# hku-mars/loam_livox

Measured on AMD Instinct MI355X. Metric: scans_per_s, higher is better.
Workload: dtype f32 points / f64 solve; 1 GPU; C2: 24k-pt Mid-40 scan vs 5M-pt corner+surface map, 10 ICP iters (fixed), k=5, Q-full; scan_points=24000, map_points=4975193, map_corner=995155, map_surf=3980038, icp_iters=10, distinct_scans_in_batch=256

## Files before the change

### loam_livox_amd/csrc/ll_reg_kernels.hip

```cpp
#include <hip/hip_runtime.h>
#include <stdlib.h>

#include "ll_reg_query.h"
#include "ll_reg_solve_common.h"

namespace ll {

#define RQ_THREADS 256
#define RQ_WAVES (RQ_THREADS / 64)
#ifndef RS_PREFETCH
#define RS_PREFETCH 2
#endif
#define RS_WAVES (RS_THREADS / 64)
#define HASH_EMPTY 0xffffffffffffffffull


#ifndef LL_REG_MAPS_TU

__global__ __launch_bounds__(KB_THREADS) void reg_transform_kernel(RegDev rd, RegConst rc, int skip_kinds)
{
    const int b = blockIdx.y, kind = blockIdx.z;
    if ((skip_kinds >> kind) & 1) return;
    const RegState *st = rd.state + b;
    if (st->done) return;
// ... 429 lines not shown
#define FAST_MAXK (FAST_MAX_BLOCKS / RS_THREADS)
#define HT_SIZE 16384
#define HT_PART 6144
#define DD_BM_WORDS 16384
#define DD_CB_LOG2 11
#define DD_CB_SIZE (1 << DD_CB_LOG2)
#define DD_EX_SIZE 4096
#define DD_MAX_COLL 900
#define DD2_WORDS 16384
#define DD2_SLOTS (DD2_WORDS * 16)
#define DD2B_WORDS 8192
#define DD2B_SLOTS (DD2B_WORDS * 16)
#define DD2_LIST 2048
#define SEL_BINS 4096
#define SEL_CAND 1024


template <int NK>
__device__ __forceinline__ void inlier_threshold_regs(const double (&l1r)[NK], int total, unsigned long long *s_table, SolveShared &sh,
                                                      const RegConst &rc)
{
    static_assert(NK <= 64 && NK <= FAST_MAXK, "register tile of the fast paths (one bit per entry in the 64-bit masks)");
    const int tid = threadIdx.x;
    LL_T0(t_dd);
    unsigned long long first_mask = 0;
    {
        int my = 0;
        unsigned int *bmA = (unsigned int *)s_table;
        unsigned int *bmB = bmA + DD2_WORDS;
        unsigned long long *dl = (unsigned long long *)(bmB + DD2B_WORDS);
        {
            uint4 *z = (uint4 *)s_table;
            for (int e = tid; e < (DD2_WORDS + DD2B_WORDS) / 4; e += RS_THREADS) z[e] = make_uint4(0u, 0u, 0u, 0u);
            if (tid == 0) sh.n_cand = 0;
        }
        __syncthreads();
        const int kt = (total + RS_THREADS - 1) / RS_THREADS;
        auto slot_a = [](unsigned long long key) -> unsigned int {
            unsigned int h = (unsigned int)key * 0x9E3779B1u;
            h ^= h >> 15;
            h += (unsigned int)(key >> 32) * 0x85EBCA77u;
            h ^= h >> 13;
            return h & (DD2_SLOTS - 1);
        };
        auto slot_b = [](unsigned long long key) -> unsigned int {
            unsigned int h2 = ((unsigned int)(key >> 32) * 0xC2B2AE3Du) ^ ((unsigned int)key * 0x27D4EB2Fu);
            return (h2 ^ (h2 >> 16)) & (DD2B_SLOTS - 1);
        };
        unsigned long long valid_mask = 0, cont_mask = 0;
#pragma unroll
        for (int k = 0; k < NK; k++) {
            if (k >= kt) continue;
            const double l1 = l1r[k];
            const bool valid = l1 >= 0.0;
            const unsigned int slot = slot_a((unsigned long long)__double_as_longlong(l1));
            const unsigned int bit0 = valid ? (1u << ((slot & 15u) * 2u)) : 0u;
            const unsigned int old = atomicOr(&bmA[slot >> 4], bit0);
            atomicOr(&bmA[slot >> 4], (old & bit0) << 1);
            if (valid) valid_mask |= 1ull << k;
        }
        __syncthreads();
#pragma unroll
        for (int k = 0; k < NK; k++) {
            if (k >= kt) continue;
            const unsigned long long key = (unsigned long long)__double_as_longlong(l1r[k]);
            const unsigned int slot = slot_a(key);
            const bool contested = ((valid_mask >> k) & 1ull) && ((bmA[slot >> 4] >> ((slot & 15u) * 2u)) & 2u);
            const unsigned int h2 = slot_b(key);
            const unsigned int bit0 = contested ? (1u << ((h2 & 15u) * 2u)) : 0u;
            const unsigned int old = atomicOr(&bmB[h2 >> 4], bit0);
            atomicOr(&bmB[h2 >> 4], (old & bit0) << 1);
            if (contested) cont_mask |= 1ull << k;
        }
        __syncthreads();
        unsigned long long twice_mask = 0;
#pragma unroll
        for (int k = 0; k < NK; k++) {
            if (k >= kt) continue;
            const unsigned int h2 = slot_b((unsigned long long)__double_as_longlong(l1r[k]));
            if (((cont_mask >> k) & 1ull) && ((bmB[h2 >> 4] >> ((h2 & 15u) * 2u)) & 2u)) twice_mask |= 1ull << k;
        }
        my = __popcll(valid_mask & ~twice_mask);
        first_mask = valid_mask & ~twice_mask;
        int my_pos[2] = {-1, -1};
        int n_twice = __popcll(twice_mask);
        if (twice_mask) {
            int got = 0;
#pragma unroll
            for (int k = 0; k < NK; k++) {
                if (!((twice_mask >> k) & 1ull)) continue;
                const int pos = atomicAdd(&sh.n_cand, 1);
                if (pos < DD2_LIST) dl[pos] = (unsigned long long)__double_as_longlong(l1r[k]);
                if (got < 2) my_pos[got] = pos;
                got++;
            }
        }
        const int over = block_sum_int(n_twice > 2 ? 1 : 0, sh);
        const int n_list = sh.n_cand;
        if (n_list <= DD2_LIST && over == 0) {
            if (twice_mask) {
                int got = 0;
#pragma unroll
                for (int k = 0; k < NK; k++) {
                    if (!((twice_mask >> k) & 1ull)) continue;
                    const int pos = my_pos[got < 2 ? got : 1];
                    got++;
                    const unsigned long long key = (unsigned long long)__double_as_longlong(l1r[k]);
                    bool dup = false;
                    for (int j = 0; j < pos; j++) dup |= (dl[j] == key);
                    if (!dup) {
                        first_mask |= 1ull << k;
                        my++;
                    }
                }
            }
        } else {
            first_mask = 0;
            my = 0;
            const int rounds = (total + HT_PART - 1) / HT_PART;
            for (int rnd = 0; rnd < rounds; rnd++) {
                __syncthreads();
                for (int e = tid; e < HT_SIZE; e += RS_THREADS) s_table[e] = HASH_EMPTY;
                __syncthreads();
#pragma unroll
                for (int k = 0; k < NK; k++) {
                    const double l1 = l1r[k];
                    if (!(l1 >= 0.0)) continue;
                    const unsigned long long key = (unsigned long long)__double_as_longlong(l1);
                    const unsigned long long hk = hash64(key);
                    if ((int)((hk >> 40) % (unsigned long long)rounds) != rnd) continue;
                    unsigned int h = (unsigned int)hk & (HT_SIZE - 1);
                    for (;;) {
                        const unsigned long long old = atomicCAS(&s_table[h], HASH_EMPTY, key);
                        if (old == HASH_EMPTY) {
                            first_mask |= (1ull << k);
                            my++;
                            break;
                        }
                        if (old == key) break;
                        h = (h + 1u) & (HT_SIZE - 1);
                    }
                }
            }
        }
        const int nu = block_sum_int(my, sh);
        if (tid == 0) {
            sh.n_unique = nu;
            sh.sel_prefix = 0ull;
            int target = (int)(rc.inlier_ratio * (double)nu);
            if (target > nu - 1) target = nu - 1;
            sh.sel_rank = target;
        }
        __syncthreads();
    }
    LL_TACC(3, t_dd);
    LL_T0(t_sel);
    if (sh.n_unique > 0) {
        int *bins = (int *)s_table;
        unsigned long long *cand = s_table + SEL_BINS / 2;
        double kmin = INFINITY, kmax = -INFINITY;
#pragma unroll
        for (int k = 0; k < NK; k++)
            if (first_mask & (1ull << k)) {
                kmin = fmin(kmin, l1r[k]);
                kmax = fmax(kmax, l1r[k]);
            }
        for (int off = 32; off > 0; off >>= 1) {
            kmin = fmin(kmin, __shfl_down(kmin, off));
            kmax = fmax(kmax, __shfl_down(kmax, off));
        }
        if ((tid & 63) == 0) {
            sh.red[tid >> 6][0] = kmin;
            sh.red[tid >> 6][1] = kmax;
        }
        for (int e = tid; e < SEL_BINS; e += RS_THREADS) bins[e] = 0;
        __syncthreads();
        double lo = sh.red[0][0], hi = sh.red[0][1];
        for (int w = 1; w < RS_WAVES; w++) {
            lo = fmin(lo, sh.red[w][0]);
            hi = fmax(hi, sh.red[w][1]);
        }
        const double scale = (hi > lo) ? (double)(SEL_BINS - 1) / (hi - lo) : 0.0;
#pragma unroll
        for (int k = 0; k < NK; k++)
            if (first_mask & (1ull << k)) {
                int bi = (int)((l1r[k] - lo) * scale);
                bi = bi < 0 ? 0 : (bi > SEL_BINS - 1 ? SEL_BINS - 1 : bi);
                atomicAdd(&bins[bi], 1);
            }
        __syncthreads();
        {
            const int per = SEL_BINS / RS_THREADS;
            const int lane = tid & 63, wave = tid >> 6;
            int part = 0;
            for (int e = 0; e < per; e++) part += bins[tid * per + e];
            int incl = part;
#pragma unroll
            for (int off = 1; off < 64; off <<= 1) {
                const int y = __shfl_up(incl, off);
                if (lane >= off) incl += y;
            }
            if (lane == 63) sh.isum[wave] = incl;
            if (tid == 0) sh.n_cand = 0;
            __syncthreads();
            int below = incl - part;
            for (int w = 0; w < wave; w++) below += sh.isum[w];
            const int rank = sh.sel_rank;
            __syncthreads();
            const bool last_thread = tid == RS_THREADS - 1;
            if ((rank >= below && rank < below + part) || (last_thread && rank >= below + part)) {
                int cum = below, bi = tid * per;
                for (; bi < tid * per + per - 1; bi++) {
                    if (cum + bins[bi] > rank) break;
                    cum += bins[bi];
                }
                sh.sel_bin = bi;
                sh.sel_rank = rank - cum;
                sh.sel_cnt = bins[bi];
            }
            __syncthreads();
        }
        if (sh.sel_cnt <= SEL_CAND) {
            const int sel_bin = sh.sel_bin;
#pragma unroll
            for (int k = 0; k < NK; k++)
                if (first_mask & (1ull << k)) {
                    int bi = (int)((l1r[k] - lo) * scale);
                    bi = bi < 0 ? 0 : (bi > SEL_BINS - 1 ? SEL_BINS - 1 : bi);
                    if (bi == sel_bin) cand[atomicAdd(&sh.n_cand, 1)] = (unsigned long long)__double_as_longlong(l1r[k]);
                }
            __syncthreads();
            const int m = sh.n_cand;
            for (int i = tid; i < m; i += RS_THREADS) {
                const unsigned long long ki = cand[i];
                int rk = 0;
                for (int j = 0; j < m; j++) rk += (cand[j] < ki) ? 1 : 0;
                if (rk == sh.sel_rank) sh.sel_prefix = ki;
            }
            __syncthreads();
        } else {
            const int sel_bin = sh.sel_bin;
            if (tid == 0) sh.sel_prefix = 0ull;
            __syncthreads();
            for (int pass = 0; pass < 8; pass++) {
                const int shift = 56 - 8 * pass;
                for (int e = tid; e < 256; e += RS_THREADS) sh.hist[e] = 0;
                __syncthreads();
                const unsigned long long prefix = sh.sel_prefix;
#pragma unroll
                for (int k = 0; k < NK; k++) {
                    if (!(first_mask & (1ull << k))) continue;
                    int bi = (int)((l1r[k] - lo) * scale);
                    bi = bi < 0 ? 0 : (bi > SEL_BINS - 1 ? SEL_BINS - 1 : bi);
                    if (bi != sel_bin) continue;
                    const unsigned long long key = (unsigned long long)__double_as_longlong(l1r[k]);
                    if (pass == 0 || (key >> (shift + 8)) == prefix) atomicAdd(&sh.hist[(int)((key >> shift) & 255ull)], 1);
                }
                __syncthreads();
                if (tid == 0) {
                    int rank = sh.sel_rank, d = 0, cum = 0;
                    for (d = 0; d < 256; d++) {
                        if (cum + sh.hist[d] > rank) break;
                        cum += sh.hist[d];
                    }
                    if (d > 255) d = 255;
                    sh.sel_rank = rank - cum;
                    sh.sel_prefix = (prefix << 8) | (unsigned long long)d;
                }
                __syncthreads();
            }
        }
        if (tid == 0) sh.thr = fmax(rc.inliner_dis, __longlong_as_double((long long)sh.sel_prefix));
    } else {
        if (tid == 0) sh.thr = rc.inliner_dis;
    }
    __syncthreads();
    LL_TACC(4, t_sel);
}

struct BlkRegs {
    float4 f;
    double a0, a1, a2, v0, v1, v2;
};

__device__ __forceinline__ void load_blk(const RegDev &rd, size_t sb, const double *av, int slot, BlkRegs &r)
{
    r.f = gload_f4(rd.blk_f + sb + slot);
    av_load(av, rd.cap, slot, slot < rd.cap_c, r.a0, r.a1, r.a2, r.v0, r.v1, r.v2);
}





#define PT_SLOTS 8192
#define PT_MAX_PROBE 192
#define PT_LDS_BYTES 155648
#define PT_TCAP (PT_LDS_BYTES / 32)
#define LL_LINE_CACHE_MAX 1024
#define PT_EMPTY_A 0xffffffffffffffffull
#define PT_EMPTY_B 0xffffffffu
#define PT_PRIVATE 0xffffu
#define PT_INACTIVE 0xfffeu

struct PtSlot {
    unsigned long long a;
    unsigned int b;
    unsigned int id;
};

__device__ __forceinline__ unsigned short gload_u16(const unsigned short *p) { return *(const LL_AS_GLOBAL unsigned short *)p; }

__device__ __forceinline__ unsigned int pt_hash(unsigned int p0, unsigned int p1, unsigned int p2)
{
    unsigned int h = p0 * 0x9E3779B1u;
    h ^= h >> 15;
    h += p1 * 0x85EBCA77u;
    h ^= h >> 13;
    h += p2 * 0xC2B2AE3Du;
    h ^= h >> 16;
    return h;
}

template <int MAX_PROBE = PT_MAX_PROBE>
__device__ __forceinline__ unsigned int pt_insert(LL_AS_LDS PtSlot *ht, unsigned int p0, unsigned int p1, unsigned int p2)
{
    const unsigned long long A = ((unsigned long long)p0 << 32) | (unsigned long long)p1;
    const unsigned int hh = pt_hash(p0, p1, p2);
    unsigned int h = hh & (PT_SLOTS - 1);
    const unsigned int step = ((hh >> 13) | 1u) & (PT_SLOTS - 1);
    for (int probe = 0; probe < MAX_PROBE; probe++) {
        unsigned long long a = __hip_atomic_load(&ht[h].a, __ATOMIC_RELAXED, __HIP_MEMORY_SCOPE_WORKGROUP);
        unsigned int bb = __hip_atomic_load(&ht[h].b, __ATOMIC_RELAXED, __HIP_MEMORY_SCOPE_WORKGROUP);
        if (a == A && bb == p2) return h;
        if (a == PT_EMPTY_A) {
            if (__hip_atomic_compare_exchange_strong(&ht[h].a, &a, A, __ATOMIC_RELAXED, __ATOMIC_RELAXED, __HIP_MEMORY_SCOPE_WORKGROUP)) a = A;
        }
        if (a == A) {
            if (bb == PT_EMPTY_B) {
                if (__hip_atomic_compare_exchange_strong(&ht[h].b, &bb, p2, __ATOMIC_RELAXED, __ATOMIC_RELAXED, __HIP_MEMORY_SCOPE_WORKGROUP)) bb = p2;
            }
            if (bb == p2) return h;
        }
        h = (h + step) & (PT_SLOTS - 1);
    }
    return PT_PRIVATE;
}

template <bool SCALED = false>
__device__ __forceinline__ void pt_plane(const f4 *map_pts, const double *pose_last, unsigned int i0, unsigned int i1, unsigned int i2, int4 &ob, int4 &oc)
{
    const f4 m0 = gload_pt(map_pts + i0), m1 = gload_pt(map_pts + i1), m2 = gload_pt(map_pts + i2);
    const double pa[3] = {(double)m0.x, (double)m0.y, (double)m0.z};
    const double pb[3] = {(double)m1.x, (double)m1.y, (double)m1.z};
    const double pc[3] = {(double)m2.x, (double)m2.y, (double)m2.z};
    double a_out[3] = {0.0, 0.0, 0.0}, v_out[3] = {0.0, 0.0, 0.0};
    (void)block_plane(pose_last, pa, pb, pc, a_out, v_out);
    if (SCALED) {
        double m_[3], beta_;
        plane_scale(v_out, a_out[0], m_, &beta_);
        v_out[0] = m_[0], v_out[1] = m_[1], v_out[2] = m_[2], a_out[0] = beta_;
    }
    ob = make_int4(__double2loint(v_out[0]), __double2hiint(v_out[0]), __double2loint(v_out[1]), __double2hiint(v_out[1]));
    oc = make_int4(__double2loint(v_out[2]), __double2hiint(v_out[2]), __double2loint(a_out[0]), __double2hiint(a_out[0]));
}

__device__ __forceinline__ int4 *pt_table_global(const RegDev &rd, int b, int g, bool grouped)
{
    return rd.pl_tab + ((size_t)b * rd.tab_cap + (grouped ? (size_t)g * (rd.tab_cap / LL_GRP) : 0)) * 2;
}

#define PT_MAP_OFF (PT_SLOTS * 16)
template <bool GROUPED>
__device__ __noinline__ unsigned long long census_and_plane_table(const RegDev &rd, const RegConst &rc, const f4 *map_pts, int b, const RegState *st,
                                                                  int nC, int nS, uint4 *s_raw, SolveShared &sh)
{
    const int tid = threadIdx.x, lane = tid & 63, wave = tid >> 6;
    constexpr int G = GROUPED ? LL_GRP : 1, GS = G * RS_THREADS;
    const int g = GROUPED ? sh.grp_g : 0;
    const int p0 = g * RS_THREADS + tid;
    const int kp = (nS + GS - 1) / GS;
    const int nSp = (nS + RS_THREADS - 1) / RS_THREADS * RS_THREADS;
    const int totp = nSp + nC;
    const size_t sb = (size_t)b * rd.cap;
    LL_AS_LDS PtSlot *ht = (LL_AS_LDS PtSlot *)s_raw;
    LL_AS_LDS unsigned short *slot_of_id = (LL_AS_LDS unsigned short *)((LL_AS_LDS char *)s_raw + PT_MAP_OFF);
    LL_T0(t_census);
    for (int e = tid; e < PT_SLOTS; e += RS_THREADS) lds_store_i4((int4 *)s_raw + e, make_int4(-1, -1, -1, -1));
    if (tid == 0) sh.pt_priv = 0;
    __syncthreads();
    const int4 *nn = rd.nn + sb + rd.cap_c;
    const unsigned char *flag0 = rd.blk_flag0 + sb;
    unsigned short *ids = rd.blk_id + (size_t)b * rd.cap_s;
    unsigned long long act = 0;
    int na = 0, nca = 0, nsa = 0;
    for (int k0 = 0; k0 * RS_THREADS < totp; k0 += 8) {
        LL_T0(t_trip);
        unsigned char fl8[8];
        int4 t8[GROUPED ? 1 : 8];
#pragma unroll
        for (int u = 0; u < 8; u++) {
            const int j = tid + (k0 + u) * RS_THREADS;
            const int jc = j < totp ? j : 0;
            const size_t src = jc < nS ? (size_t)rd.cap_c + jc : (jc >= nSp ? (size_t)(jc - nSp) : (size_t)rd.cap_c);
            fl8[u] = gload_u8(flag0 + src);
            if (!GROUPED) t8[u] = gload_i4(nn + (j < nS ? j : 0));
        }
        if (GROUPED) {
            const int j = tid + (k0 + g) * RS_THREADS;
            t8[0] = gload_i4(nn + (j < nS ? j : 0));
        }
        unsigned int h8[GROUPED ? 1 : 8];
#ifdef LL_SOLVE_TIMING
        if (fl8[0] == 255 && t8[0].x == -12345) act |= 1ull << 63;
        LL_TACC(10, t_trip);
        LL_T0(t_ins);
#endif
#pragma unroll
        for (int u = 0; u < 8; u++) {
            const int j = tid + (k0 + u) * RS_THREADS;
            const unsigned char fl = (j < totp && (j < nS || j >= nSp)) ? fl8[u] : (unsigned char)0;
            const bool active = (fl & BLK_ACTIVE) != 0;
            if (active) {
                act |= 1ull << (k0 + u);
                na++;
            }
            if (fl & 8) {
                if (j >= nSp) nca++; else nsa++;
            }
            if (!GROUPED || u == g) {
                const int4 t = t8[GROUPED ? 0 : u];
                const unsigned int h = (active && j < nS) ? pt_insert(ht, (unsigned int)t.x, (unsigned int)t.y, (unsigned int)t.z) : PT_INACTIVE;
                if (h == PT_PRIVATE) atomicAdd(&sh.pt_priv, 1);
                h8[GROUPED ? 0 : u] = h;
            }
        }
#pragma unroll
        for (int u = 0; u < 8; u++) {
            const int j = tid + (k0 + u) * RS_THREADS;
            if ((!GROUPED || u == g) && j < nS) gstore_u16(ids + j, (unsigned short)h8[GROUPED ? 0 : u]);
        }
#ifdef LL_SOLVE_TIMING
        LL_TACC(11, t_ins);
#endif
    }
    LL_T0(t_sums);
    {
        const unsigned long long tot = block_sum_u64((unsigned long long)na | ((unsigned long long)nca << 20) | ((unsigned long long)nsa << 40), sh);
        na = (int)(tot & 0xfffffull);
        nca = (int)((tot >> 20) & 0xfffffull);
        nsa = (int)((tot >> 40) & 0xfffffull);
    }
    if (rc.subsample_seed && na > rc.max_blocks) {
        int kept = 0;
        for (int k = 0; k * RS_THREADS < totp; k++) {
            if (!((act >> k) & 1ull)) continue;
            const int j = tid + k * RS_THREADS;
            const int jref = j >= nSp ? j - nSp : nC + j;
            if (subsample_drop_block(rc.subsample_seed, st->icp_iters, jref, na, rc.max_blocks))
                act &= ~(1ull << k);
            else
                kept++;
        }
        na = block_sum_int(kept, sh);
    }
    if (tid == 0) {
        sh.n_active = na;
        sh.n_corner_avail = nca;
        sh.n_surf_avail = nsa;
    }
    __syncthreads();
    LL_TACC(12, t_sums);
    LL_TACC(6, t_census);
    LL_T0(t_tab);
    LL_T0(t_cmp);
    constexpr int SPT = PT_SLOTS / RS_THREADS;
    unsigned int occ = 0;
#pragma unroll
    for (int i = 0; i < SPT; i++)
        if (ht[tid + i * RS_THREADS].b != PT_EMPTY_B) occ |= 1u << i;
    const int cnt = __popc(occ);
    int incl = cnt;
#pragma unroll
    for (int off = 1; off < 64; off <<= 1) {
        const int y = __shfl_up(incl, off);
        if (lane >= off) incl += y;
    }
    if (lane == 63) sh.isum[wave] = incl;
    __syncthreads();
    int base = incl - cnt, T = 0;
    for (int w = 0; w < RS_WAVES; w++) {
        if (w < wave) base += sh.isum[w];
        T += sh.isum[w];
    }
    {
        int rk = base;
#pragma unroll
        for (int i = 0; i < SPT; i++)
            if (occ & (1u << i)) {
                ht[tid + i * RS_THREADS].id = (unsigned int)rk;
                slot_of_id[rk] = (unsigned short)(tid + i * RS_THREADS);
                rk++;
            }
    }
    __syncthreads();
    LL_TACC(13, t_cmp);
    LL_T0(t_pl);
    int4 *tabG = pt_table_global(rd, b, g, GROUPED);
    double pose_last[7];
#pragma unroll
    for (int i = 0; i < 7; i++) pose_last[i] = gload_f64(st->pose_last + i);
    for (int i0 = tid; i0 < T; i0 += 4 * RS_THREADS) {
        f4 m[4][3];
#pragma unroll
        for (int u = 0; u < 4; u++) {
            const int id = i0 + u * RS_THREADS;
            const unsigned int sl = slot_of_id[id < T ? id : i0];
            const unsigned long long sa = ht[sl].a;
            const unsigned int sb2 = ht[sl].b;
            m[u][0] = gload_pt(map_pts + (unsigned int)(sa >> 32));
            m[u][1] = gload_pt(map_pts + (unsigned int)sa);
            m[u][2] = gload_pt(map_pts + sb2);
        }
#pragma unroll
        for (int u = 0; u < 4; u++) {
            const int id = i0 + u * RS_THREADS;
            const double pa[3] = {(double)m[u][0].x, (double)m[u][0].y, (double)m[u][0].z};
            const double pb[3] = {(double)m[u][1].x, (double)m[u][1].y, (double)m[u][1].z};
            const double pc[3] = {(double)m[u][2].x, (double)m[u][2].y, (double)m[u][2].z};
            double a_out[3] = {0.0, 0.0, 0.0}, v_out[3] = {0.0, 0.0, 0.0};
            (void)block_plane(pose_last, pa, pb, pc, a_out, v_out);
            {
                double m_[3], beta_;
                plane_scale(v_out, a_out[0], m_, &beta_);
                v_out[0] = m_[0], v_out[1] = m_[1], v_out[2] = m_[2], a_out[0] = beta_;
            }
            if (id < T) {
                gstore_i4(tabG + 2 * id, make_int4(__double2loint(v_out[0]), __double2hiint(v_out[0]), __double2loint(v_out[1]), __double2hiint(v_out[1])));
                gstore_i4(tabG + 2 * id + 1, make_int4(__double2loint(v_out[2]), __double2hiint(v_out[2]), __double2loint(a_out[0]), __double2hiint(a_out[0])));
            }
        }
    }
    LL_TACC(14, t_pl);
    LL_T0(t_p2);
    const int region = GROUPED ? rd.tab_cap / LL_GRP : rd.tab_cap;
    for (int k0 = 0; k0 < kp; k0 += 8) {
        unsigned short h8[8];
#pragma unroll
        for (int u = 0; u < 8; u++) {
            const int p = p0 + (k0 + u) * GS;
            h8[u] = gload_u16(ids + (p < nS ? p : 0));
        }
        unsigned int id8[8];
#pragma unroll
        for (int u = 0; u < 8; u++) {
            const unsigned int h = h8[u];
            const unsigned int sid = ht[h < PT_SLOTS ? h : 0u].id;
            id8[u] = h < PT_SLOTS ? sid : (h == PT_PRIVATE ? PT_PRIVATE : 0u);
        }
#pragma unroll
        for (int u = 0; u < 8; u++) {
            const int p = p0 + (k0 + u) * GS;
            if (p < nS) gstore_u16(ids + p, (unsigned short)id8[u]);
        }
    }
    if (sh.pt_priv > 0) {
        int npriv = 0;
        for (int k = 0; k < kp; k++) {
            const int p = p0 + k * GS;
            if (p < nS && gload_u16(ids + p) == PT_PRIVATE) npriv++;
        }
        int incl2 = npriv;
#pragma unroll
        for (int off = 1; off < 64; off <<= 1) {
            const int y = __shfl_up(incl2, off);
            if (lane >= off) incl2 += y;
        }
        __syncthreads();
        if (lane == 63) sh.isum[wave] = incl2;
        __syncthreads();
        int pid = incl2 - npriv;
        for (int w = 0; w < wave; w++) pid += sh.isum[w];
        for (int k = 0; k < kp; k++) {
            const int p = p0 + k * GS;
            if (p >= nS || gload_u16(ids + p) != PT_PRIVATE) continue;
            const unsigned int id = (unsigned int)(region - 1 - pid);
            pid++;
            const int4 t = gload_i4(nn + p);
            int4 ob, oc;
            pt_plane<true>(map_pts, pose_last, (unsigned int)t.x, (unsigned int)t.y, (unsigned int)t.z, ob, oc);
            gstore_i4(tabG + 2 * id, ob);
            gstore_i4(tabG + 2 * id + 1, oc);
            gstore_u16(ids + p, (unsigned short)id);
        }
    }
    __threadfence_block();
    __syncthreads();
    const int Tl = T < PT_TCAP ? T : PT_TCAP;
    int4 *s_tab = (int4 *)s_raw;
    for (int e0 = tid; e0 < 2 * Tl; e0 += 8 * RS_THREADS) {
        int4 v8[8];
#pragma unroll
        for (int u = 0; u < 8; u++) {
            const int e = e0 + u * RS_THREADS;
            v8[u] = gload_i4(tabG + (e < 2 * Tl ? e : e0));
        }
#pragma unroll
        for (int u = 0; u < 8; u++) {
            const int e = e0 + u * RS_THREADS;
            if (e < 2 * Tl) lds_store_i4(s_tab + e, v8[u]);
        }
    }
    if (tid == 0) {
        int nl = 0;
        if (!rc.no_line_cache && T <= PT_TCAP && sh.pt_priv == 0) {
            int mine = GROUPED ? nC - g * RS_THREADS : nC;
            const int cap = GROUPED ? RS_THREADS : LL_LINE_CACHE_MAX;
            mine = mine < 0 ? 0 : (mine > cap ? cap : mine);
            const int room = (PT_LDS_BYTES / 16 - 2 * Tl) / 4;
            nl = mine < room ? mine : room;
        }
        const int kc = (PT_LDS_BYTES / 16 - 2 * Tl - 4 * nl) / RS_THREADS;
        sh.pt_T = sh.pt_priv > 0 ? PT_TCAP + 1 : T;
        sh.pt_Tl = Tl;
        sh.pt_kc = kc < kp ? kc : kp;
        sh.pt_nl = nl;
    }
    __syncthreads();
    LL_TACC(15, t_p2);
    LL_TACC(8, t_tab);
    return act;
}

__device__ __forceinline__ void plane_table_reload(const RegDev &rd, int b, bool grouped, uint4 *s_raw, SolveShared &sh)
{
    const int4 *tabG = pt_table_global(rd, b, grouped ? sh.grp_g : 0, grouped);
    int4 *s_tab = (int4 *)s_raw;
    const int n = 2 * sh.pt_Tl;
    for (int e0 = threadIdx.x; e0 < n; e0 += 8 * RS_THREADS) {
        int4 v8[8];
#pragma unroll
        for (int u = 0; u < 8; u++) {
            const int e = e0 + u * RS_THREADS;
            v8[u] = gload_i4(tabG + (e < n ? e : e0));
        }
#pragma unroll
        for (int u = 0; u < 8; u++) {
            const int e = e0 + u * RS_THREADS;
            if (e < n) lds_store_i4(s_tab + e, v8[u]);
        }
    }
    __syncthreads();
}

struct Rec3 {
    int fx, fy, fz;
    unsigned int id;
};
struct Pl3 {
    int4 b, c;
};

#define LL3_LOAD(R, K)                                                                             \
    {                                                                                              \
        if (FROM_CACHE_) {                                                                         \
            const int kc_ = (K) < kc ? (K) : kc - 1;                                               \
            const int4 c_ = lds_load_i4(cache + tid + kc_ * RS_THREADS);                           \
            R.fx = c_.x;                                                                           \
            R.fy = c_.y;                                                                           \
            R.fz = c_.z;                                                                           \
            R.id = (unsigned int)c_.w;                                                             \
        } else {                                                                                   \
            const int pp_ = p0 + (K) * GS;                                                         \
            const int pc_ = pp_ < nS ? pp_ : 0;                                                    \
            float fx_, fy_, fz_;                                                                   \
            gload_f3(feat + pc_, fx_, fy_, fz_);                                                   \
            R.id = gload_u16(ids + pc_);                                                           \
            R.fx = __float_as_int(fx_);                                                            \
            R.fy = __float_as_int(fy_);                                                            \
            R.fz = __float_as_int(fz_);                                                            \
        }                                                                                          \
    }
#define LL3_PLANE(Q, R)                                                                            \
    {                                                                                              \
        if (TAB_LDS || R.id < (unsigned int)Tl) {                                                  \
            Q.b = lds_load_i4(tabL + 2 * R.id);                                                    \
            Q.c = lds_load_i4(tabL + 2 * R.id + 1);                                                \
        } else {                                                                                   \
            Q.b = gload_i4(tabG + 2 * R.id);                                                       \
            Q.c = gload_i4(tabG + 2 * R.id + 1);                                                   \
        }                                                                                          \
    }
#define LL3_USE(R, Q, K)                                                                                   \
    if ((K) < KE_) {                                                                                       \
        const int pp_ = p0 + (K) * GS;                                                                     \
        if (FILL && (K) < kc) lds_store_i4(cache + tid + (K) * RS_THREADS, make_int4(R.fx, R.fy, R.fz, (int)R.id)); \
        if (pp_ < nS && ((act >> (g + G * (K))) & 1ull)) {  \
            const double f[3] = {(double)__int_as_float(R.fx), (double)__int_as_float(R.fy), (double)__int_as_float(R.fz)}; \
            const double v[3] = {__hiloint2double(Q.b.y, Q.b.x), __hiloint2double(Q.b.w, Q.b.z), __hiloint2double(Q.c.y, Q.c.x)}; \
            const double beta_ = __hiloint2double(Q.c.w, Q.c.z);                                           \
            plane_accumulate_scaled(R_, t_, f, v, beta_, huber_a, acc);                                    \
            if (L1OUT) gstore_f64(l1_planes + pp_, plane_l1_scaled(R_, t_, f, v, beta_, huber_a, q_last)); \
        }                                                                                                  \
    }
#define LL3_PIPE(FROM_CACHE, KB, KE)                                   \
    {                                                                  \
        constexpr bool FROM_CACHE_ = FROM_CACHE;                       \
        const int KB_ = (KB), KE_ = (KE);                              \
        if (KB_ < KE_) {                                               \
            Rec3 r0, r1, r2, r3, r4;                                   \
            Pl3 q0, q1, q2, q3, q4;                                    \
            LL3_LOAD(r0, KB_)                                          \
            LL3_LOAD(r1, KB_ + 1)                                      \
            LL3_LOAD(r2, KB_ + 2)                                      \
            LL3_LOAD(r3, KB_ + 3)                                      \
            LL3_PLANE(q0, r0)                                          \
            for (int k = KB_; k < KE_; k += 5) {                       \
                LL3_LOAD(r4, k + 4)                                    \
                LL3_PLANE(q1, r1)                                      \
                LL3_USE(r0, q0, k)                                     \
                LL3_LOAD(r0, k + 5)                                    \
                LL3_PLANE(q2, r2)                                      \
                LL3_USE(r1, q1, k + 1)                                 \
                LL3_LOAD(r1, k + 6)                                    \
                LL3_PLANE(q3, r3)                                      \
                LL3_USE(r2, q2, k + 2)                                 \
                LL3_LOAD(r2, k + 7)                                    \
                LL3_PLANE(q4, r4)                                      \
                LL3_USE(r3, q3, k + 3)                                 \
                LL3_LOAD(r3, k + 8)                                    \
                LL3_PLANE(q0, r0)                                      \
                LL3_USE(r4, q4, k + 4)                                 \
            }                                                          \
        }                                                              \
    }

template <bool FILL, bool L1OUT, bool GROUPED>
__device__ __noinline__ void solver_eval3(const RegDev &rd, int b, int nC, int nS, const double *x, double huber_a, unsigned long long act,
                                          uint4 *s_raw, const double *q_last_g, SolveShared &sh)
{
    constexpr int DEBLUR = 0;
    const int tid = threadIdx.x, lane = tid & 63, wave = tid >> 6;
    double q_last[4] = {0.0, 0.0, 0.0, 1.0};
    if (L1OUT) {
        q_last[0] = q_last_g[0];
        q_last[1] = q_last_g[1];
        q_last[2] = q_last_g[2];
        q_last[3] = q_last_g[3];
    }
    double *l1_planes = rd.blk_l1 + (size_t)b * rd.cap + rd.cap_c;
    double *l1_lines = rd.blk_l1 + (size_t)b * rd.cap;
    LL_CTX_DECL(x)
    double acc[LL_NACC];
#pragma unroll
    for (int i = 0; i < LL_NACC; i++) acc[i] = 0.0;
    constexpr int G = GROUPED ? LL_GRP : 1, GS = G * RS_THREADS;
    const int g = GROUPED ? sh.grp_g : 0;
    const int p0 = g * RS_THREADS + tid;
    const int Tl = sh.pt_Tl, kc = sh.pt_kc;
    const int kp = (nS + GS - 1) / GS;
    const int4 *tabL = (const int4 *)s_raw;
    int4 *cache = (int4 *)s_raw + 2 * Tl;
    const int4 *tabG = pt_table_global(rd, b, g, GROUPED);
    const unsigned short *ids = rd.blk_id + (size_t)b * rd.cap_s;
    const float4 *feat = rd.surf_feat + (size_t)b * rd.feat_stride_s;
    if (sh.pt_T <= PT_TCAP) {
        constexpr bool TAB_LDS = true;
        if (!FILL) LL3_PIPE(true, 0, kc)
        LL3_PIPE(false, FILL ? 0 : kc, kp)
    } else {
        constexpr bool TAB_LDS = false;
        if (!FILL) LL3_PIPE(true, 0, kc)
        LL3_PIPE(false, FILL ? 0 : kc, kp)
    }
    plane_unfold2(acc);
#ifdef LL_EXP_MOMENT_EVAL
    {
        double xacc[LL_NACC];
#pragma unroll
        for (int i = 0; i < LL_NACC; i++) xacc[i] = 0.0;
        int n_lin = 0;
        for (int k0 = 0; k0 < kp; k0 += 8) {
            float fx8[8], fy8[8], fz8[8];
            unsigned int id8[8];
#pragma unroll
            for (int u = 0; u < 8; u++) {
                const int pp = p0 + (k0 + u) * GS;
                const int pc = pp < nS ? pp : 0;
                gload_f3(feat + pc, fx8[u], fy8[u], fz8[u]);
                id8[u] = gload_u16(ids + pc);
            }
#pragma unroll
            for (int u = 0; u < 8; u++) {
                const int k = k0 + u, pp = p0 + k * GS;
                const unsigned int idl = id8[u] < (unsigned int)Tl ? id8[u] : 0u;
                const int4 qb = lds_load_i4(tabL + 2 * idl), qc = lds_load_i4(tabL + 2 * idl + 1);
                const double f[3] = {(double)fx8[u], (double)fy8[u], (double)fz8[u]};
                const double m[3] = {__hiloint2double(qb.y, qb.x), __hiloint2double(qb.w, qb.z), __hiloint2double(qc.y, qc.x)};
                const double beta = __hiloint2double(qc.w, qc.z);
                const double q0 = R_[0] * f[0] + R_[1] * f[1] + R_[2] * f[2] + t_[0], q1 = R_[3] * f[0] + R_[4] * f[1] + R_[5] * f[2] + t_[1],
                             q2 = R_[6] * f[0] + R_[7] * f[1] + R_[8] * f[2] + t_[2];
                const double e = m[0] * q0 + m[1] * q1 + m[2] * q2 - beta;
                if (k < kp && pp < nS && ((act >> (g + G * k)) & 1ull) && e * e > huber_a * huber_a) n_lin++;
            }
        }
        const double *mom = rd.blk_av + (size_t)b * 6 * rd.cap + 2 * (size_t)rd.cap_c;
        for (int id = tid; id < sh.pt_T && id < Tl; id += RS_THREADS) {
            const int4 qb = lds_load_i4(tabL + 2 * id), qc = lds_load_i4(tabL + 2 * id + 1);
            const double m[3] = {__hiloint2double(qb.y, qb.x), __hiloint2double(qb.w, qb.z), __hiloint2double(qc.y, qc.x)};
            const double beta = __hiloint2double(qc.w, qc.z);
            double mo[10];
#pragma unroll
            for (int i = 0; i < 10; i += 2) {
                const double2 v2 = gload_d2(reinterpret_cast<const double2 *>(mom + (size_t)id * 10 + i));
                mo[i] = v2.x;
                mo[i + 1] = v2.y;
            }
            const double ms[3] = {R_[0] * m[0] + R_[3] * m[1] + R_[6] * m[2], R_[1] * m[0] + R_[4] * m[1] + R_[7] * m[2], R_[2] * m[0] + R_[5] * m[1] + R_[8] * m[2]};
            const double bs = m[0] * t_[0] + m[1] * t_[1] + m[2] * t_[2] - beta;
            const double N = mo[0], S1[3] = {mo[1], mo[2], mo[3]};
            const double S2[9] = {mo[4], mo[5], mo[6], mo[5], mo[7], mo[8], mo[6], mo[8], mo[9]};
            double u[3];
#pragma unroll
            for (int i = 0; i < 3; i++) u[i] = S2[3 * i] * ms[0] + S2[3 * i + 1] * ms[1] + S2[3 * i + 2] * ms[2];
            const double l1 = ms[0] * S1[0] + ms[1] * S1[1] + ms[2] * S1[2];
            xacc[27] += 0.5 * (ms[0] * u[0] + ms[1] * u[1] + ms[2] * u[2] + 2.0 * bs * l1 + N * bs * bs);
            const double w[3] = {u[0] + bs * S1[0], u[1] + bs * S1[1], u[2] + bs * S1[2]};
            double gt[3], sx[3];
            cross3(w, ms, gt);
            cross3(S1, ms, sx);
            const double gb = l1 + N * bs;
#pragma unroll
            for (int i = 0; i < 3; i++) {
                xacc[21 + i] += 2.0 * gt[i];
                xacc[24 + i] += gb * ms[i];
            }
            double A[9];
#pragma unroll
            for (int r = 0; r < 3; r++) {
                const double row[3] = {S2[3 * r], S2[3 * r + 1], S2[3 * r + 2]};
                double c[3];
                cross3(row, ms, c);
                A[3 * r] = c[0], A[3 * r + 1] = c[1], A[3 * r + 2] = c[2];
            }
#pragma unroll
            for (int c = 0; c < 3; c++) {
                const double col[3] = {A[c], A[3 + c], A[6 + c]};
                double h[3];
                cross3(ms, col, h);
#pragma unroll
                for (int r = 0; r <= c; r++) xacc[hidx(r, c)] += 4.0 * h[r];
            }
#pragma unroll
            for (int i = 0; i < 3; i++)
#pragma unroll
                for (int j = 0; j < 3; j++) {
                    xacc[hidx(i, 3 + j)] += 2.0 * sx[i] * ms[j];
                    if (j >= i) xacc[hidx(3 + i, 3 + j)] += N * ms[i] * ms[j];
                }
        }
        double xs = (double)n_lin;
#pragma unroll
        for (int i = 0; i < LL_NACC; i++) xs += xacc[i];
        if (xs == 1.2345678e300) acc[27] += xs;
    }
#endif
    {
        const size_t sb = (size_t)b * rd.cap;
        const double *av = rd.blk_av + (size_t)b * 6 * rd.cap;
        const int kpl = (nS + RS_THREADS - 1) / RS_THREADS;
        const int nl = sh.pt_nl;
        int4 *lc = (int4 *)s_raw + (PT_LDS_BYTES / 16 - 4 * nl);
        int k = 0;
        for (int l = p0; l < nC; l += GS, k++) {
            if (!((act >> (kpl + g + G * k)) & 1ull)) continue;
            BlkRegs br;
            const int j = GROUPED ? (k == 0 ? tid : nl) : l;
            if (!FILL && j < nl) {
                const int4 c0 = lds_load_i4(lc + j), c1 = lds_load_i4(lc + nl + j), c2 = lds_load_i4(lc + 2 * nl + j), c3 = lds_load_i4(lc + 3 * nl + j);
                br.f = make_float4(__int_as_float(c0.x), __int_as_float(c0.y), __int_as_float(c0.z), __int_as_float(c0.w));
                br.a0 = __hiloint2double(c1.y, c1.x);
                br.v0 = __hiloint2double(c1.w, c1.z);
                br.v1 = __hiloint2double(c2.y, c2.x);
                br.v2 = __hiloint2double(c2.w, c2.z);
                br.a1 = __hiloint2double(c3.y, c3.x);
                br.a2 = __hiloint2double(c3.w, c3.z);
            } else {
                load_blk(rd, sb, av, l, br);
                if (FILL && j < nl) {
                    lds_store_i4(lc + j, make_int4(__float_as_int(br.f.x), __float_as_int(br.f.y), __float_as_int(br.f.z), __float_as_int(br.f.w)));
                    lds_store_i4(lc + nl + j, make_int4(__double2loint(br.a0), __double2hiint(br.a0), __double2loint(br.v0), __double2hiint(br.v0)));
                    lds_store_i4(lc + 2 * nl + j, make_int4(__double2loint(br.v1), __double2hiint(br.v1), __double2loint(br.v2), __double2hiint(br.v2)));
                    lds_store_i4(lc + 3 * nl + j, make_int4(__double2loint(br.a1), __double2hiint(br.a1), __double2loint(br.a2), __double2hiint(br.a2)));
                }
            }
            const double a[3] = {br.a0, br.a1, br.a2};
            const double v[3] = {br.v0, br.v1, br.v2};
            LL_CTX_ACCUM(BLK_LINE, br.f, a, v, huber_a, acc);
            if (L1OUT) {
                double l1;
                LL_CTX_L1(l1, BLK_LINE, br.f, a, v, huber_a, q_last);
                l1_lines[l] = l1;
            }
        }
    }
    if (__ballot(act != 0ull) != 0ull) {
        wave_sum_acc(acc, sh.red[wave], lane);
    } else if (lane < LL_NACC) {
        sh.red[wave][lane] = 0.0;
    }
    __syncthreads();
    if (tid < LL_NACC) {
        double s = 0.0;
        for (int w = 0; w < RS_WAVES; w++) s += sh.red[w][tid];
        sh.sum[tid] = s;
    }
    __syncthreads();
    if (GROUPED) {
        LL_T0(t_grp);
        group_reduce<L1OUT>(rd, b, sh);
        LL_TACC(9, t_grp);
    }
}
#undef LL3_LOAD
#undef LL3_PLANE
#undef LL3_USE
#undef LL3_PIPE


#ifndef LL_REG_MAPS_TU
__global__ __launch_bounds__(64) void debug_quintic_kernel(const double *args, int n, double *out_seq, double *out_wave)
{
// ... 525 lines not shown
```

Before: 52280 scans/s.

## Keep hash slots in registers and write plane table directly to LDS

During insertion the per-point hash slot indices are packed into registers instead of being written to global memory and read back in the id-remap pass. The hash-table entries are cached in registers before the LDS is overwritten, and the plane-fitting loop now runs after the id remap. It writes results straight into the LDS table as well as global memory, which removes the separate global-to-LDS reload loop. The cost is much higher register pressure from large per-thread arrays, plus reliance on FAST_MAX_BLOCKS bounds for the register indexing.

Result: faster. 52810 scans/s (median of 6 runs) (+1.0%).

```diff
diff --git a/loam_livox_amd/csrc/ll_reg_kernels.hip b/loam_livox_amd/csrc/ll_reg_kernels.hip
--- a/loam_livox_amd/csrc/ll_reg_kernels.hip
+++ b/loam_livox_amd/csrc/ll_reg_kernels.hip
@@ -755,6 +755,7 @@
 #define PT_EMPTY_B 0xffffffffu
 #define PT_PRIVATE 0xffffu
 #define PT_INACTIVE 0xfffeu
+#define PT_NTRIP (FAST_MAX_BLOCKS / RS_THREADS / 8)
 
 struct PtSlot {
     unsigned long long a;
@@ -847,6 +848,10 @@
     unsigned short *ids = rd.blk_id + (size_t)b * rd.cap_s;
     unsigned long long act = 0;
     int na = 0, nca = 0, nsa = 0;
+    constexpr int NHREG = GROUPED ? PT_NTRIP / 2 : PT_NTRIP * 4;
+    unsigned int hreg[NHREG];
+#pragma unroll
+    for (int i = 0; i < NHREG; i++) hreg[i] = PT_INACTIVE | (PT_INACTIVE << 16);
     for (int k0 = 0; k0 * RS_THREADS < totp; k0 += 8) {
         LL_T0(t_trip);
         unsigned char fl8[8];
@@ -889,10 +894,15 @@
             }
         }
 #pragma unroll
-        for (int u = 0; u < 8; u++) {
-            const int j = tid + (k0 + u) * RS_THREADS;
-            if ((!GROUPED || u == g) && j < nS) gstore_u16(ids + j, (unsigned short)h8[GROUPED ? 0 : u]);
-        }
+        for (int t = 0; t < PT_NTRIP; t++)
+            if ((k0 >> 3) == t) {
+                if constexpr (GROUPED) {
+                    hreg[t / 2] = (t & 1) ? ((hreg[t / 2] & 0xffffu) | (h8[0] << 16)) : ((hreg[t / 2] & 0xffff0000u) | h8[0]);
+                } else {
+#pragma unroll
+                    for (int i = 0; i < 4; i++) hreg[4 * t + i] = h8[2 * i] | (h8[2 * i + 1] << 16);
+                }
+            }
 #ifdef LL_SOLVE_TIMING
         LL_TACC(11, t_ins);
 #endif
@@ -958,63 +968,46 @@
     }
     __syncthreads();
     LL_TACC(13, t_cmp);
-    LL_T0(t_pl);
+    LL_T0(t_p2);
     int4 *tabG = pt_table_global(rd, b, g, GROUPED);
     double pose_last[7];
 #pragma unroll
     for (int i = 0; i < 7; i++) pose_last[i] = gload_f64(st->pose_last + i);
-    for (int i0 = tid; i0 < T; i0 += 4 * RS_THREADS) {
-        f4 m[4][3];
-#pragma unroll
-        for (int u = 0; u < 4; u++) {
-            const int id = i0 + u * RS_THREADS;
-            const unsigned int sl = slot_of_id[id < T ? id : i0];
-            const unsigned long long sa = ht[sl].a;
-            const unsigned int sb2 = ht[sl].b;
-            m[u][0] = gload_pt(map_pts + (unsigned int)(sa >> 32));
-            m[u][1] = gload_pt(map_pts + (unsigned int)sa);
-            m[u][2] = gload_pt(map_pts + sb2);
-        }
-#pragma unroll
-        for (int u = 0; u < 4; u++) {
-            const int id = i0 + u * RS_THREADS;
-            const double pa[3] = {(double)m[u][0].x, (double)m[u][0].y, (double)m[u][0].z};
-            const double pb[3] = {(double)m[u][1].x, (double)m[u][1].y, (double)m[u][1].z};
-            const double pc[3] = {(double)m[u][2].x, (double)m[u][2].y, (double)m[u][2].z};
-            double a_out[3] = {0.0, 0.0, 0.0}, v_out[3] = {0.0, 0.0, 0.0};
-            (void)block_plane(pose_last, pa, pb, pc, a_out, v_out);
-            {
-                double m_[3], beta_;
-                plane_scale(v_out, a_out[0], m_, &beta_);
-                v_out[0] = m_[0], v_out[1] = m_[1], v_out[2] = m_[2], a_out[0] = beta_;
-            }
-            if (id < T) {
-                gstore_i4(tabG + 2 * id, make_int4(__double2loint(v_out[0]), __double2hiint(v_out[0]), __double2loint(v_out[1]), __double2hiint(v_out[1])));
-                gstore_i4(tabG + 2 * id + 1, make_int4(__double2loint(v_out[2]), __double2hiint(v_out[2]), __double2loint(a_out[0]), __double2hiint(a_out[0])));
-            }
-        }
-    }
-    LL_TACC(14, t_pl);
-    LL_T0(t_p2);
     const int region = GROUPED ? rd.tab_cap / LL_GRP : rd.tab_cap;
-    for (int k0 = 0; k0 < kp; k0 += 8) {
-        unsigned short h8[8];
-#pragma unroll
-        for (int u = 0; u < 8; u++) {
-            const int p = p0 + (k0 + u) * GS;
-            h8[u] = gload_u16(ids + (p < nS ? p : 0));
-        }
-        unsigned int id8[8];
-#pragma unroll
-        for (int u = 0; u < 8; u++) {
-            const unsigned int h = h8[u];
+    if constexpr (GROUPED) {
+        unsigned int id8[PT_NTRIP];
+#pragma unroll
+        for (int u = 0; u < PT_NTRIP; u++) {
+            const unsigned int h = (hreg[u / 2] >> ((u & 1) * 16)) & 0xffffu;
             const unsigned int sid = ht[h < PT_SLOTS ? h : 0u].id;
             id8[u] = h < PT_SLOTS ? sid : (h == PT_PRIVATE ? PT_PRIVATE : 0u);
         }
 #pragma unroll
-        for (int u = 0; u < 8; u++) {
-            const int p = p0 + (k0 + u) * GS;
+        for (int u = 0; u < PT_NTRIP; u++) {
+            const int p = p0 + u * GS;
             if (p < nS) gstore_u16(ids + p, (unsigned short)id8[u]);
+        }
+    } else {
+        for (int k0 = 0; k0 < kp; k0 += 8) {
+            unsigned int w4[4] = {0u, 0u, 0u, 0u};
+#pragma unroll
+            for (int t = 0; t < PT_NTRIP; t++)
+                if ((k0 >> 3) == t) {
+#pragma unroll
+                    for (int i = 0; i < 4; i++) w4[i] = hreg[4 * t + i];
+                }
+            unsigned int id8[8];
+#pragma unroll
+            for (int u = 0; u < 8; u++) {
+                const unsigned int h = (w4[u >> 1] >> ((u & 1) * 16)) & 0xffffu;
+                const unsigned int sid = ht[h < PT_SLOTS ? h : 0u].id;
+                id8[u] = h < PT_SLOTS ? sid : (h == PT_PRIVATE ? PT_PRIVATE : 0u);
+            }
+#pragma unroll
+            for (int u = 0; u < 8; u++) {
+                const int p = p0 + (k0 + u) * GS;
+                if (p < nS) gstore_u16(ids + p, (unsigned short)id8[u]);
+            }
         }
     }
     if (sh.pt_priv > 0) {
@@ -1047,23 +1040,26 @@
             gstore_u16(ids + p, (unsigned short)id);
         }
     }
-    __threadfence_block();
-    __syncthreads();
+    LL_TACC(15, t_p2);
+    LL_T0(t_pl);
+    constexpr int IPT = PT_SLOTS / RS_THREADS;
+    const int Tu = __builtin_amdgcn_readfirstlane(T);
+    unsigned long long ta[IPT];
+    unsigned int tb[IPT];
+#pragma unroll
+    for (int i = 0; i < IPT; i++) ta[i] = 0ull, tb[i] = 0u;
+#pragma unroll
+    for (int q = 0; q < IPT / 4; q++)
+        if (q * 4 * RS_THREADS < Tu) {
+#pragma unroll
+            for (int u = 0; u < 4; u++) {
+                const int id = tid + (4 * q + u) * RS_THREADS;
+                const unsigned int sl = slot_of_id[id < T ? id : 0] & (PT_SLOTS - 1);
+                ta[4 * q + u] = ht[sl].a;
+                tb[4 * q + u] = ht[sl].b;
+            }
+        }
     const int Tl = T < PT_TCAP ? T : PT_TCAP;
-    int4 *s_tab = (int4 *)s_raw;
-    for (int e0 = tid; e0 < 2 * Tl; e0 += 8 * RS_THREADS) {
-        int4 v8[8];
-#pragma unroll
-        for (int u = 0; u < 8; u++) {
-            const int e = e0 + u * RS_THREADS;
-            v8[u] = gload_i4(tabG + (e < 2 * Tl ? e : e0));
-        }
-#pragma unroll
-        for (int u = 0; u < 8; u++) {
-            const int e = e0 + u * RS_THREADS;
-            if (e < 2 * Tl) lds_store_i4(s_tab + e, v8[u]);
-        }
-    }
     if (tid == 0) {
         int nl = 0;
         if (!rc.no_line_cache && T <= PT_TCAP && sh.pt_priv == 0) {
@@ -1080,7 +1076,57 @@
         sh.pt_nl = nl;
     }
     __syncthreads();
-    LL_TACC(15, t_p2);
+    int4 *s_tab = (int4 *)s_raw;
+#pragma unroll 1
+    for (int q = 0; q * 4 * RS_THREADS < Tu; q++) {
+        unsigned long long a4[4] = {0ull, 0ull, 0ull, 0ull};
+        unsigned int b4[4] = {0u, 0u, 0u, 0u};
+#pragma unroll
+        for (int t = 0; t < IPT / 4; t++)
+            if (q == t) {
+#pragma unroll
+                for (int u = 0; u < 4; u++) a4[u] = ta[4 * t + u], b4[u] = tb[4 * t + u];
+            }
+        const int i0 = tid + q * 4 * RS_THREADS;
+        if (i0 < T) {
+            f4 m[4][3];
+#pragma unroll
+            for (int u = 0; u < 4; u++) {
+                const int id = i0 + u * RS_THREADS;
+                const unsigned long long sa = id < T ? a4[u] : a4[0];
+                const unsigned int sb2 = id < T ? b4[u] : b4[0];
+                m[u][0] = gload_pt(map_pts + (unsigned int)(sa >> 32));
+                m[u][1] = gload_pt(map_pts + (unsigned int)sa);
+                m[u][2] = gload_pt(map_pts + sb2);
+            }
+#pragma unroll
+            for (int u = 0; u < 4; u++) {
+                const int id = i0 + u * RS_THREADS;
+                const double pa[3] = {(double)m[u][0].x, (double)m[u][0].y, (double)m[u][0].z};
+                const double pb[3] = {(double)m[u][1].x, (double)m[u][1].y, (double)m[u][1].z};
+                const double pc[3] = {(double)m[u][2].x, (double)m[u][2].y, (double)m[u][2].z};
+                double a_out[3] = {0.0, 0.0, 0.0}, v_out[3] = {0.0, 0.0, 0.0};
+                (void)block_plane(pose_last, pa, pb, pc, a_out, v_out);
+                {
+                    double m_[3], beta_;
+                    plane_scale(v_out, a_out[0], m_, &beta_);
+                    v_out[0] = m_[0], v_out[1] = m_[1], v_out[2] = m_[2], a_out[0] = beta_;
+                }
+                const int4 ob = make_int4(__double2loint(v_out[0]), __double2hiint(v_out[0]), __double2loint(v_out[1]), __double2hiint(v_out[1]));
+                const int4 oc = make_int4(__double2loint(v_out[2]), __double2hiint(v_out[2]), __double2loint(a_out[0]), __double2hiint(a_out[0]));
+                if (id < Tl) {
+                    lds_store_i4(s_tab + 2 * id, ob);
+                    lds_store_i4(s_tab + 2 * id + 1, oc);
+                }
+                if (id < T) {
+                    gstore_i4(tabG + 2 * id, ob);
+                    gstore_i4(tabG + 2 * id + 1, oc);
+                }
+            }
+        }
+    }
+    __syncthreads();
+    LL_TACC(14, t_pl);
     LL_TACC(8, t_tab);
     return act;
 }
```
